# Malfoy/Brisk

Hardware: AMD Instinct MI355X
Metric: distinct k-mers indexed/sec (k=63,m=21) (higher is better)
Workload: dtype u64; 1 GPU; 1x MI355X: 50M synthetic 150 bp reads per GPU, k=63 m=21 b=14, uint8 counts, 15x coverage; reads_per_gpu=50000000, total_reads=50000000, part_bits=24, genome_len=500000000, parallelism=single GPU

## Files before the change

brisk_amd/csrc/brisk_insert.hip:

```cpp
#ifndef ARENA_CHUNK
#define ARENA_CHUNK 16384u
#endif
#ifndef INSERT_SLOTS
#define INSERT_SLOTS 8192u
#endif
#ifndef WI_WAVES_PER_EU
#define WI_WAVES_PER_EU 4
#endif
#ifdef BRISK_PHASE_PROF
__device__ unsigned long long g_phase[16];
#define PHASE_DECL unsigned long long ph_acc[12] = {0, 0, 0, 0, 0, 0, 0, 0, 0, 0, 0, 0}; unsigned long long ph_last = __builtin_amdgcn_s_memtime(); u32 dbg_cnt[16] = {0, 0, 0, 0, 0, 0, 0, 0, 0, 0, 0, 0, 0, 0, 0, 0};
#define PHASE(i) { const unsigned long long t_ = __builtin_amdgcn_s_memtime(); ph_acc[i] += t_ - ph_last; ph_last = t_; }
__device__ unsigned long long g_cnt[16];
#define PHASE_FLUSH { PHASE(10) if (threadIdx.x == 0) { _Pragma("unroll") for (int q_ = 0; q_ < 12; q_++) atomicAdd(&g_phase[q_], ph_acc[q_]); \
                                                         _Pragma("unroll") for (int q_ = 0; q_ < 16; q_++) atomicAdd(&g_cnt[q_], (unsigned long long)dbg_cnt[q_]); } }
#define CNT(i, v) dbg_cnt[i] += (v);
#else
#define PHASE_DECL
#define PHASE(i)
#define PHASE_FLUSH
#define CNT(i, v)
#endif
struct IndexDev {
    u64* keys;
// ... 152 lines not shown
    for (u32 it = 0; it < NI; it++) {
        const u32 i = it * 64 + lane;
        const u32 r = rix[it];
        const u64* c = s_rec + r * (NW ? NW + 1 : P.stride);
        const u64 hdr = c[NW ? NW : P.nw];
        const u32 j = i < ninst ? i - s_pref[r] : 0;
        const u128x key = make_key(P, hdr_bucket(hdr), record_kmer_lds<NW>(P, c, hdr_n(hdr), j), hdr_idx0(hdr) + j);
        klo[it] = key.lo;
        khi[it] = key.hi;
        hh[it] = hash_key32(key) & (tsize - 1);
        mult[it] = count8<SAT>(s_rmult[r]) << WI_CNT_SHIFT;
        if (i < ninst) {
            s_key[2 * i] = key.lo;
            s_key[2 * i + 1] = key.hi;
        }
    }
    wave_sync();
    u32 pending = 0;
#pragma unroll
    for (u32 it = 0; it < NI; it++)
        if (it * 64 + lane < ninst) pending |= 1u << it;
    while (__any(pending != 0)) {
        u32 old[NI];
#pragma unroll
        for (u32 it = 0; it < NI; it++) {
            old[it] = EMPTY_SLOT;
            if (pending >> it & 1) old[it] = atomicCAS(&s_tab[hh[it]], EMPTY_SLOT, (it * 64 + lane) | mult[it]);
        }
        u64 olo[NI], ohi[NI];
#pragma unroll
        for (u32 it = 0; it < NI; it++) {
            const u32 oi = old[it] == EMPTY_SLOT ? 0 : (old[it] & WI_IDX_MASK);
            olo[it] = s_key[2 * oi];
            ohi[it] = s_key[2 * oi + 1];
        }
#pragma unroll
        for (u32 it = 0; it < NI; it++) {
            if (pending >> it & 1) {
                if (old[it] == EMPTY_SLOT) {
                    pending &= ~(1u << it);
                } else if (olo[it] == klo[it] && ohi[it] == khi[it]) {
                    atomicAdd(&s_tab[hh[it]], mult[it]);
                    pending &= ~(1u << it);
                } else {
                    hh[it] = (hh[it] + 1) & (tsize - 1);
                }
            }
        }
    }
}

template <u32 NW>
struct RecGeom {
    static constexpr u32 CW = 2 * NW + 1;
    static constexpr u32 RS = 2 * NW + 3;
    static constexpr u32 INFO = 2 * NW + 1;
};
template <u32 NW>
__device__ __forceinline__ void store_rec_words(u32* dst, const RecRegs& rr, u32 info) {
    const u64 c0 = rr.w0, c1 = NW > 1 ? rr.w1 : 0, c2 = NW > 2 ? rr.w2 : 0, c3 = NW > 3 ? rr.w3 : 0;
    const u64 s0 = c0 << 6, s1 = (c1 << 6) | (c0 >> 58), s2 = (c2 << 6) | (c1 >> 58), s3 = (c3 << 6) | (c2 >> 58);
    const u32 top = (u32)((NW == 1 ? c0 : NW == 2 ? c1 : NW == 3 ? c2 : c3) >> 58);
    dst[0] = (u32)s0;
    dst[1] = (u32)(s0 >> 32);
    if (NW > 1) { dst[2] = (u32)s1; dst[3] = (u32)(s1 >> 32); }
    if (NW > 2) { dst[4] = (u32)s2; dst[5] = (u32)(s2 >> 32); }
    if (NW > 3) { dst[6] = (u32)s3; dst[7] = (u32)(s3 >> 32); }
    dst[2 * NW] = top;
    dst[RecGeom<NW>::INFO] = info;
    dst[RecGeom<NW>::INFO + 1] = 0;
}
template <u32 NIMAX>
struct LaneInst {
    u64 klo[NIMAX], khi[NIMAX];
    u32 hh[NIMAX];
    u32 won;
};
template <u32 NW, u32 KB, u32 SHIFT>
__device__ __forceinline__ void cut_key(const u32* base, u32 i, u32 ninst, u64* lo_out, u64* hi_out) {
    constexpr u32 INFO = RecGeom<NW>::INFO, KBITS = 2 * KB + 6;
    const u32 info = base[INFO];
    const u32 j = i < ninst ? i - (info & 0x3ffu) : 0;
    const u32 n = (info >> 10) & 0xffu;
    const u32 s = 2 * (n - 1 - j);
    const u32* wp = base + (s >> 5);
    const u32 sh = s & 31;
    const u32 w0 = wp[0], w1 = wp[1], w2 = wp[2], w3 = wp[3], w4 = wp[4];
    u32 k0 = __builtin_amdgcn_alignbit(w1, w0, sh), k1 = __builtin_amdgcn_alignbit(w2, w1, sh);
    u32 k2 = __builtin_amdgcn_alignbit(w3, w2, sh), k3 = __builtin_amdgcn_alignbit(w4, w3, sh);
    k0 = (k0 & ~0x3fu) | (((info >> 18) & 0xffu) + j);
    constexpr u32 m0 = KBITS >= 32 ? ~0u : (1u << KBITS) - 1, m1 = KBITS >= 64 ? ~0u : KBITS <= 32 ? 0u : (1u << (KBITS - 32)) - 1;
    constexpr u32 m2 = KBITS >= 96 ? ~0u : KBITS <= 64 ? 0u : (1u << (KBITS - 64)) - 1, m3 = KBITS >= 128 ? ~0u : KBITS <= 96 ? 0u : (1u << (KBITS - 96)) - 1;
    k0 &= m0; k1 &= m1; k2 &= m2; k3 &= m3;
    u64 lo = ((u64)k1 << 32) | k0, hi = ((u64)k3 << 32) | k2;
    if (SHIFT) {
        const u64 rl = (info >> 26) & ((1u << SHIFT) - 1);
        if (KBITS >= 64) hi |= rl << (KBITS - 64);
        else {
            lo |= rl << KBITS;
            if (KBITS + SHIFT > 64) hi |= rl >> (64 - KBITS);
        }
    }
    *lo_out = lo;
    *hi_out = hi;
}
template <u32 NI, u32 NW, u32 KB, u32 SHIFT, u32 NIMAX>
__device__ __forceinline__ void expand_words_distinct(u32 lane, u32 ninst, const u32* s_rw, const uint8_t* s_irec, LaneInst<NIMAX>& li) {
    static_assert(NI <= NIMAX, "instances per lane");
    u32 rix[NI];
    u32 won = 0;
#pragma unroll
    for (u32 it = 0; it < NI; it++) {
        const u32 i = it * 64 + lane;
        rix[it] = s_irec[i < ninst ? i : 0];
    }
#pragma unroll
    for (u32 it = 0; it < NI; it++) {
        const u32 i = it * 64 + lane;
        cut_key<NW, KB, SHIFT>(s_rw + rix[it] * RecGeom<NW>::RS, i, ninst, &li.klo[it], &li.khi[it]);
        if (i < ninst) won |= 1u << it;
    }
    li.won = won;
}
template <u32 NI, u32 NW, u32 KB, u32 SHIFT, u32 NIMAX, bool FOLD, bool SAT>
__device__ __forceinline__ void expand_and_dedupe_words(u32 lane, u32 ninst, u32 tsize, const u32* s_rw, const uint8_t* s_irec, const uint8_t* s_imult,
                                                        const u32* s_rmult, u64* s_key, u32* s_tab, u32* dbg_rounds, LaneInst<NIMAX>& li) {
    constexpr u32 RS = RecGeom<NW>::RS, KBITS = 2 * KB + 6;
    static_assert(KBITS + SHIFT <= 128 && SHIFT <= 6, "entry key: [routing id low bits | compacted k-mer | idx']");
    static_assert(NI <= NIMAX, "instances per lane");
    u64 (&klo)[NIMAX] = li.klo;
    u64 (&khi)[NIMAX] = li.khi;
    u32 (&hh)[NIMAX] = li.hh;
    u32 mult[NI];
    u32 rix[NI];
    u32 won = 0;
#pragma unroll
    for (u32 it = 0; it < NI; it++) {
        const u32 i = it * 64 + lane;
        rix[it] = s_irec[i < ninst ? i : 0];
    }
#pragma unroll
    for (u32 it = 0; it < NI; it++) {
        const u32 i = it * 64 + lane;
        u64 lo, hi;
        cut_key<NW, KB, SHIFT>(s_rw + rix[it] * RS, i, ninst, &lo, &hi);
        klo[it] = lo;
        khi[it] = hi;
        hh[it] = hash_key32(mk128(lo, hi)) & (tsize - 1);
        mult[it] = FOLD ? (u32)s_imult[i < ninst ? i : 0] << WI_CNT_SHIFT : count8<SAT>(s_rmult[rix[it]]) << WI_CNT_SHIFT;
        if (i < ninst) {
            s_key[2 * i] = lo;
            s_key[2 * i + 1] = hi;
        }
    }
    wave_sync();
    for (u32 w = 0; w * 64 < tsize; w++) s_tab[w * 64 + lane] = EMPTY_SLOT;
    wave_sync();
    u32 pending = 0;
#pragma unroll
    for (u32 it = 0; it < NI; it++)
        if (it * 64 + lane < ninst) pending |= 1u << it;
    while (__any(pending != 0)) {
        *dbg_rounds += NI;
        u32 old[NI];
#pragma unroll
        for (u32 it = 0; it < NI; it++) {
            old[it] = EMPTY_SLOT;
            if (pending >> it & 1) old[it] = atomicCAS(&s_tab[hh[it]], EMPTY_SLOT, (it * 64 + lane) | mult[it]);
        }
        u64 olo[NI], ohi[NI];
#pragma unroll
        for (u32 it = 0; it < NI; it++) {
            const u32 oi = old[it] == EMPTY_SLOT ? 0 : (old[it] & WI_IDX_MASK);
            olo[it] = s_key[2 * oi];
            ohi[it] = s_key[2 * oi + 1];
        }
#pragma unroll
        for (u32 it = 0; it < NI; it++) {
            if (pending >> it & 1) {
                if (old[it] == EMPTY_SLOT) {
                    pending &= ~(1u << it);
                    won |= 1u << it;
                } else if (olo[it] == klo[it] && ohi[it] == khi[it]) {
                    atomicAdd(&s_tab[hh[it]], mult[it]);
                    pending &= ~(1u << it);
                } else {
                    hh[it] = (hh[it] + 1) & (tsize - 1);
                }
            }
        }
    }
    li.won = won;
}

#define HDR_ID_MASK 0x0000ffffffffffffull
#define HDR_HAS_MULT (1ull << 56)
__device__ __forceinline__ bool dedupe_records(u32 stride, const RecRegs& rr, u32 my_mult, u32 nrec, u32 lane, const u64* s_rec, u32* s_rtab, u32* s_rmult) {
    s_rtab[lane] = EMPTY_SLOT;
    s_rtab[lane + 64] = EMPTY_SLOT;
    s_rmult[lane] = my_mult;
    wave_sync();
    bool dup = false;
    if (lane < nrec) {
        const u64 k1 = stride == 2 ? HDR_ID_MASK : ~0ull, k2 = stride == 3 ? HDR_ID_MASK : ~0ull, k3 = stride == 4 ? HDR_ID_MASK : ~0ull,
                  k4 = stride == 5 ? HDR_ID_MASK : ~0ull;
        const u64 w1 = rr.w1 & k1, w2 = rr.w2 & k2, w3 = rr.w3 & k3, w4 = rr.w4 & k4;
        const u64 z = rr.w0 ^ ((w1 << 17) | (w1 >> 47)) ^ ((w2 << 31) | (w2 >> 33)) ^ ((w3 << 47) | (w3 >> 17)) ^ w4;
        u32 h = ((((u32)z ^ (u32)(z >> 32)) * 0x9E3779B1u) >> 20) & (2 * WI_MAX_REC - 1);
        for (;;) {
            const u32 o = atomicCAS(&s_rtab[h], EMPTY_SLOT, lane);
            if (o == EMPTY_SLOT) break;
            const u64* oc = s_rec + o * stride;
            bool same = oc[0] == rr.w0 && (oc[1] & k1) == w1;
            if (stride > 2) same = same && (oc[2] & k2) == w2;
            if (stride > 3) same = same && (oc[3] & k3) == w3;
            if (stride > 4) same = same && (oc[4] & k4) == w4;
            if (same) {
                atomicAdd(&s_rmult[o], my_mult);
                dup = true;
                break;
            }
            h = (h + 1) & (2 * WI_MAX_REC - 1);
        }
    }
    return dup;
}

#ifndef WI_FOLD_TRIPS
#define WI_FOLD_TRIPS 16u
#endif
struct FoldFrame {
    W4 u, m;
    u32 rid;
    u32 rng;
    u32 s;
};
template <u32 NW, u32 KB>
__device__ __forceinline__ FoldFrame fold_frame(const RecRegs& rr, u64 hdr, u32 n, bool valid, u32 frame_end, u32 lane) {
    FoldFrame f;
    const u32 idx0 = hdr_idx0(hdr), end = idx0 + n, top = frame_end - idx0 + KB - 1;
    const bool ok = valid && n > 0 && end <= frame_end && top <= 32 * NW;
    const u32 lo_bits = ok ? 2 * (frame_end - end) : 0, hi_bits = ok ? 2 * top : 0;
    f.m = w4_andn(w4_mask(hi_bits), w4_mask(lo_bits));
    f.u = w4_and(w4_shl(W4{rr.w0, NW > 1 ? rr.w1 : 0, NW > 2 ? rr.w2 : 0, NW > 3 ? rr.w3 : 0}, lo_bits), f.m);
    f.rid = hdr_bucket(hdr);
    f.rng = idx0 | (end << 8);
    f.s = ok ? (n << 6) | (63 - lane) : 0;
    return f;
}
__device__ __forceinline__ u64 readlane64(u64 v, u32 a) {
    return ((u64)(u32)__builtin_amdgcn_readlane((int)(v >> 32), (int)a) << 32) | (u32)__builtin_amdgcn_readlane((int)v, (int)a);
}
template <u32 KB, u32 CW>
__device__ __forceinline__ u32 fold_core(const W4& u) {
    constexpr u32 LO = 2 * CW, N = 2 * (KB - CW), WI = LO / 64, BI = LO % 64;
    static_assert(CW < KB && N <= 28 && LO + N <= 256, "the core: the minimizer's nucleotides that are not cut out, m - b of them");
    const u64 w[5] = {u.w0, u.w1, u.w2, u.w3, 0};
    u64 v = w[WI] >> BI;
    if (BI + N > 64) v |= w[WI + 1] << (64 - BI);
    return (u32)v & ((1u << N) - 1);
}
template <u32 NW, bool DETECT = false>
__device__ __forceinline__ bool fold_records(const FoldFrame& f, u32 nrec, u32 lane, u32* lead, u32* off, u32* trips, u32 ck = 0, bool unsure = false, bool* clean = nullptr) {
    u32 sv = lane < nrec ? f.s : 0;
    bool folded = false;
    u32 dirty = unsure;
    *lead = lane;
    *off = 0;
    for (u32 t = 0; t < WI_FOLD_TRIPS; t++) {
        const u32 smax = (u32)__builtin_amdgcn_readlane((int)wave_incl_max_scan(sv), 63);
        if (smax == 0) break;
        *trips += 1;
        const u32 a = 63 - (smax & 63);
        const u32 rid_a = (u32)__builtin_amdgcn_readlane((int)f.rid, (int)a), rng_a = (u32)__builtin_amdgcn_readlane((int)f.rng, (int)a);
        const u32 i0 = f.rng & 0xffu, e = f.rng >> 8, i0a = rng_a & 0xffu, ea = rng_a >> 8;
#ifdef BRISK_NO_RECORD_FOLD
        bool in = sv != 0 && rid_a == f.rid && i0a == i0 && ea == e;
#else
        bool in = sv != 0 && rid_a == f.rid && i0a <= i0 && e <= ea;
#endif
        bool same = (readlane64(f.u.w0, a) & f.m.w0) == f.u.w0;
        if (NW > 1) same = same & ((readlane64(f.u.w1, a) & f.m.w1) == f.u.w1);
        if (NW > 2) same = same & ((readlane64(f.u.w2, a) & f.m.w2) == f.u.w2);
        if (NW > 3) same = same & ((readlane64(f.u.w3, a) & f.m.w3) == f.u.w3);
        in = in && same;
        if (in) {
            sv = 0;
            if (lane != a) {
                folded = true;
                *lead = a;
                *off = i0 - i0a;
            }
        }
        if (DETECT) {
            const u32 differs = ck ^ (u32)__builtin_amdgcn_readlane((int)ck, (int)a);
            const u32 meets = ((i0 - ea) & (i0a - e)) >> 31;
            dirty |= (differs == 0 && sv != 0) ? meets : 0u;
        }
    }
    if (DETECT) *clean = !__any((dirty | sv) != 0);
    return folded;
}

template <u32 MAXI, u32 NW, u32 KB, u32 SHIFT, bool SAT, bool LISTED = false>
__device__ __forceinline__ void insert_body(const BriskParams& PP, const RecSrc& src, const PartDesc* __restrict__ desc, u32 n_touched_all, const IndexDev& ix,
                                            u32* __restrict__ work_counter, const u32* __restrict__ list = nullptr, const u32* __restrict__ n_list = nullptr) {
    const u32 n_touched = LISTED ? min(*n_list, n_touched_all) : n_touched_all;
    u64* const rec = src.rec;
    BriskParams P = PP;
    if (NW) {
        P.nw = NW;
        P.stride = NW + 1;
        P.kb = KB;
        P.shift = SHIFT;
    }
    constexpr u32 TABLE = 2 * MAXI, TS = TABLE / 64, NI = MAXI / 64;
    constexpr u32 KW = NW ? (2 * KB + 6 + SHIFT <= 64 ? 1u : 2u) : 0u;
    constexpr bool FOLD = NW >= 3 && MAXI == WI_MAX_INST;
    static_assert(MAXI % 256 == 0 && MAXI <= 1024, "chunk size: whole 32-bit words of record marks per lane, 10-bit instance index");
    constexpr u32 REC_U64 = WI_MAX_REC * 5 > MAXI / 2 ? WI_MAX_REC * 5 : MAXI / 2;
    static_assert(NW == 0 || (WI_MAX_REC * RecGeom<NW ? NW : 1>::RS + 4) * 4 <= REC_U64 * 8, "shifted record words must fit the record buffer");
    constexpr bool TAB_OVER_REC = NW && TABLE * 4 <= REC_U64 * 8;
    constexpr u32 OFF_REC = 16 * MAXI, OFF_TAB = TAB_OVER_REC ? OFF_REC : OFF_REC + 8 * REC_U64, OFF_RTAB = TAB_OVER_REC ? OFF_REC + 8 * REC_U64 : OFF_TAB + 4 * TABLE;
    constexpr u32 OFF_RMULT = OFF_RTAB + 4 * 2 * WI_MAX_REC, OFF_IREC = OFF_RMULT + 4 * WI_MAX_REC, OFF_PREF = OFF_IREC + MAXI;
    constexpr u32 LDS_BYTES = NW ? OFF_PREF : OFF_PREF + 4 * (WI_MAX_REC + 1) + 4;
    __shared__ __attribute__((aligned(16))) unsigned char s_mem[LDS_BYTES];
    u64* s_key = (u64*)s_mem;
    u32* s_idiff = (u32*)s_mem;
    u64* s_rec = (u64*)(s_mem + OFF_REC);
    u32* s_rw = (u32*)s_rec;
    u32* s_tab = (u32*)(s_mem + OFF_TAB);
    u32* s_list = (u32*)s_rec;
    u32* s_rtab = (u32*)(s_mem + OFF_RTAB);
    u32* s_rmult = (u32*)(s_mem + OFF_RMULT);
    uint8_t* s_irec = s_mem + OFF_IREC;
    uint8_t* s_imult = s_mem + OFF_RTAB;
    static_assert(NW == 0 || MAXI <= 4 * 2 * WI_MAX_REC, "instance multiplicities fit the record table's bytes");
    u32* s_pref = (u32*)(s_mem + (NW ? 0 : OFF_PREF));

    const u32 lane = threadIdx.x;
    PHASE_DECL
    unsigned long long acur = ix.slot_cur[blockIdx.x], aend = ix.slot_end[blockIdx.x], garbage = 0;
    const u32 kbits = 2 * P.kb + 6;

    for (;;) {
        u32 t0 = 0;
        if (lane == 0) t0 = atomicAdd(work_counter, WI_BATCH);
        t0 = (u32)__builtin_amdgcn_readfirstlane((int)t0);
        if (t0 >= n_touched) break;
        const u32 t_end = min(t0 + WI_BATCH, n_touched);
        PartDesc d = desc[LISTED ? list[t0] : t0];
        RecRegs rr = load_part_recs(P, src, d.part, d.r_begin, d.r_begin, min(d.n_rec, (u32)WI_MAX_REC), lane);

        for (u32 t = t0; t < t_end; t++) {
            const u32 tn = t + 1;
            PartDesc dn{};
            if (tn < t_end) dn = desc[LISTED ? list[tn] : tn];
#define NEXT_PARTITION                                                                                                  \
    {                                                                                                                   \
        d = dn;                                                                                                         \
        if (tn < t_end) rr = load_part_recs(P, src, d.part, d.r_begin, d.r_begin, min(d.n_rec, (u32)WI_MAX_REC), lane); \
    }

            asm volatile("" ::"v"(rr.w0), "v"(rr.w1), "v"(rr.w2), "v"(rr.w3), "v"(rr.w4));
            do {
            if (ix.huge_at && d.n_inst > ix.huge_at) break;
            CNT(0, 1)
            const u32 part = d.part;
            u32 r_end = d.r_begin + d.n_rec;
            u32 n_exist = d.n_exist;
            u32 inst_left = d.n_inst;
            unsigned long long off = d.off;
            u32 cap = d.cap;
            u32 bm0 = 0, bm1 = 0;

            bool collapsed = false;
            if (MAXI > WI_MAX_INST && !src.bin_cap && d.n_rec > 2 * WI_MAX_REC) {
                u32 wr = d.r_begin;
                for (u32 rd = d.r_begin; rd < r_end; rd += WI_MAX_REC) {
                    const u32 avail = min(r_end - rd, (u32)WI_MAX_REC);
                    if (rd != d.r_begin) rr = load_rec_regs(P, rec, rd, avail, lane);
                    wave_sync();
                    if (lane < avail) {
                        u64* dst = s_rec + lane * P.stride;
                        dst[0] = rr.w0;
                        dst[1] = rr.w1;
                        if (P.stride > 2) dst[2] = rr.w2;
                        if (P.stride > 3) dst[3] = rr.w3;
                        if (P.stride > 4) dst[4] = rr.w4;
                    }
                    const u64 hdr_c = P.stride == 2 ? rr.w1 : P.stride == 3 ? rr.w2 : P.stride == 4 ? rr.w3 : rr.w4;
                    const u32 mult_c = (hdr_c & HDR_HAS_MULT) ? (u32)(hdr_c >> 48) & 0xffu : 1u;
                    const bool dup = dedupe_records(P.stride, rr, mult_c, avail, lane, s_rec, s_rtab, s_rmult);
                    wave_sync();
                    const bool keep = lane < avail && !dup;
                    const unsigned long long bal = __ballot(keep);
                    if (keep) {
                        u64* dst = rec + (u64)(wr + (u32)__popcll(bal & lanes_below(lane))) * P.stride;
                        const u64 keep_id = HDR_ID_MASK, mult = ((u64)count8<SAT>(s_rmult[lane]) << 48) | HDR_HAS_MULT;
                        dst[0] = rr.w0;
                        dst[1] = P.stride == 2 ? (rr.w1 & keep_id) | mult : rr.w1;
                        if (P.stride > 2) dst[2] = P.stride == 3 ? (rr.w2 & keep_id) | mult : rr.w2;
                        if (P.stride > 3) dst[3] = P.stride == 4 ? (rr.w3 & keep_id) | mult : rr.w3;
                        if (P.stride > 4) dst[4] = (rr.w4 & keep_id) | mult;
                    }
                    wr += (u32)__popcll(bal);
                }
                collapsed = true;
                r_end = wr;
                __builtin_amdgcn_fence(__ATOMIC_SEQ_CST, "workgroup");
                rr = load_rec_regs(P, rec, d.r_begin, min(r_end - d.r_begin, (u32)WI_MAX_REC), lane);
            }

            for (u32 rc = d.r_begin; rc < r_end;) {
                PHASE(0)
                CNT(1, 1)
                const u32 avail = min(r_end - rc, (u32)WI_MAX_REC);
                if (rc != d.r_begin) rr = load_part_recs(P, src, part, d.r_begin, rc, avail, lane);
                wave_sync();
                if (!FOLD && lane < avail) {
                    u64* dst = s_rec + lane * P.stride;
                    dst[0] = rr.w0;
                    dst[1] = rr.w1;
                    if (P.stride > 2) dst[2] = rr.w2;
                    if (P.stride > 3) dst[3] = rr.w3;
                    if (P.stride > 4) dst[4] = rr.w4;
                }
                const u64 my_hdr = P.stride == 2 ? rr.w1 : P.stride == 3 ? rr.w2 : P.stride == 4 ? rr.w3 : rr.w4;
                const u32 raw_n = lane < avail ? hdr_n(my_hdr) : 0;
                const u32 my_mult = (my_hdr & HDR_HAS_MULT) ? (u32)(my_hdr >> 48) & 0xffu : 1u;
                const u32 x0 = wave_incl_scan(raw_n, lane);
                const u32 rawfit = (u32)__popcll(__ballot(lane < avail && x0 <= MAXI));
                u32 nrec = avail, my_n = 0, x = 0, ninst = 0;
                u32 lead = lane, lead_off = 0, dbg_trips = 0;
                FoldFrame ff{};
                const u32 info_hi = (raw_n << 10) | (hdr_idx0(my_hdr) << 18) | ((hdr_bucket(my_hdr) & ((1u << SHIFT) - 1)) << 26);
                if (FOLD) {
                    ff = fold_frame<NW ? NW : 1, KB>(rr, my_hdr, raw_n, lane < avail, P.suff_reduc + P.w + 1, lane);
                    if (lane < avail) store_rec_words<NW ? NW : 1>(s_rw + lane * RecGeom<NW ? NW : 1>::RS, rr, 0);
                }
                for (int attempt = 0;; attempt++) {
                    CNT(2, 1)
                    bool dup;
                    if (FOLD) dup = fold_records<NW ? NW : 1>(ff, nrec, lane, &lead, &lead_off, &dbg_trips);
                    else dup = dedupe_records(P.stride, rr, my_mult, nrec, lane, s_rec, s_rtab, s_rmult);
                    my_n = (lane < nrec && !dup) ? raw_n : 0;
                    x = wave_incl_scan(my_n, lane);
                    ninst = __shfl(x, 63, 64);
                    if (ninst <= MAXI) break;
                    const u32 fit = (u32)__popcll(__ballot(lane < nrec && x <= MAXI));
                    nrec = (attempt >= 2 || fit <= rawfit) ? rawfit : min(fit, nrec - 1);
                    wave_sync();
                }
                PHASE(1)
                const u32 raw_inst = __shfl(x0, nrec - 1, 64);
                CNT(9, raw_inst)
                CNT(10, FOLD ? (u32)__popcll(__ballot(lane < nrec && my_n == 0 && raw_n != 0)) : 0u)
                CNT(11, dbg_trips)
                CNT(12, rc == d.r_begin && d.n_rec <= WI_MAX_REC && ninst > 64 && ninst <= 128 ? 1u : 0u)
                CNT(13, rc == d.r_begin && d.n_rec <= WI_MAX_REC && ninst > 128 && ninst <= 192 ? 1u : 0u)
                CNT(14, rc == d.r_begin && d.n_rec <= WI_MAX_REC && ninst > 192 ? 1u : 0u)
                CNT(15, rc == d.r_begin && d.n_rec > WI_MAX_REC ? 1u : 0u)
                const u32 m_first = FOLD ? (u32)__shfl(x - my_n, lead, 64) + lead_off : 0u;
                u32 tsize = 128;
                while (tsize < 4 * ninst && tsize < TABLE) tsize <<= 1;
                if (!NW) {
                    s_pref[lane + 1] = x;
                    if (lane == 0) s_pref[0] = 0;
#pragma unroll
                    for (u32 w = 0; w < TS; w++)
                        if (w * 64 < tsize) s_tab[w * 64 + lane] = EMPTY_SLOT;
                }
                {
                    u32* irec32 = (u32*)s_irec;
#pragma unroll
                    for (u32 q = 0; q < MAXI / 256; q++) irec32[q * 64 + lane] = 0;
                    if (FOLD) {
#pragma unroll
                        for (u32 q = 0; q < NI; q++) s_idiff[lane * NI + q] = 0;
                    }
                    wave_sync();
                    if (my_n) s_irec[x - my_n] = (uint8_t)(lane + 1);
                    if (FOLD && lane < nrec) {
                        atomicAdd(&s_idiff[m_first], my_mult);
                        if (m_first + raw_n < ninst) atomicAdd(&s_idiff[m_first + raw_n], 0u - my_mult);
                    }
                    wave_sync();
                    u32 wv[MAXI / 256], run = 0;
#pragma unroll
                    for (u32 q = 0; q < MAXI / 256; q++) {
                        wv[q] = irec32[lane * (MAXI / 256) + q];
                        run = op_max_u32(run, op_max_u32(op_max_u32(wv[q] & 0xff, (wv[q] >> 8) & 0xff), op_max_u32((wv[q] >> 16) & 0xff, wv[q] >> 24)));
                    }
                    if (FOLD) {
                        u32 mv[NI], tot = 0;
#pragma unroll
                        for (u32 q = 0; q < NI; q++) {
                            tot += s_idiff[lane * NI + q];
                            mv[q] = tot;
                        }
                        const u32 before = wave_incl_scan(tot, lane) - tot;
                        u32* mult32 = (u32*)s_imult;
#pragma unroll
                        for (u32 q = 0; q < NI / 4; q++)
                            mult32[lane * (NI / 4) + q] = count8<SAT>(mv[4 * q] + before) | (count8<SAT>(mv[4 * q + 1] + before) << 8) |
                                                          (count8<SAT>(mv[4 * q + 2] + before) << 16) |
                                                          ((SAT ? count8<SAT>(mv[4 * q + 3] + before) : mv[4 * q + 3] + before) << 24);
                    }
                    u32 carry = wave_prev_lane(wave_incl_max_scan(run));
#pragma unroll
                    for (u32 q = 0; q < MAXI / 256; q++) {
                        const u32 b0 = op_max_u32(carry, wv[q] & 0xff), b1 = op_max_u32(b0, (wv[q] >> 8) & 0xff);
                        const u32 b2 = op_max_u32(b1, (wv[q] >> 16) & 0xff), b3 = op_max_u32(b2, wv[q] >> 24);
                        carry = b3;
                        irec32[lane * (MAXI / 256) + q] = ((b0 - 1) & 0xff) | (((b1 - 1) & 0xff) << 8) | (((b2 - 1) & 0xff) << 16) | ((b3 - 1) << 24);
                    }
                }
                wave_sync();
                PHASE(2)
                u32 dbg_r = 0;
                LaneInst<NI> li;
                li.won = 0;
                CNT(3, (ninst + 63) / 64)
                CNT(4, ninst)
                CNT(5, nrec)
                if (NW) {
                    if (FOLD && lane < nrec) s_rw[lane * RecGeom<NW ? NW : 1>::RS + RecGeom<NW ? NW : 1>::INFO] = (x - my_n) | info_hi;
                    if (!FOLD && lane < nrec) store_rec_words<NW ? NW : 1>(s_rw + lane * RecGeom<NW ? NW : 1>::RS, rr, (x - my_n) | info_hi);
                    wave_sync();
                    if (ninst <= 64) expand_and_dedupe_words<1, NW ? NW : 1, KB, SHIFT, NI, FOLD, SAT>(lane, ninst, tsize, s_rw, s_irec, s_imult, s_rmult, s_key, s_tab, &dbg_r, li);
                    else if (ninst <= 128) expand_and_dedupe_words<2, NW ? NW : 1, KB, SHIFT, NI, FOLD, SAT>(lane, ninst, tsize, s_rw, s_irec, s_imult, s_rmult, s_key, s_tab, &dbg_r, li);
                    else if (ninst <= 192) expand_and_dedupe_words<3, NW ? NW : 1, KB, SHIFT, NI, FOLD, SAT>(lane, ninst, tsize, s_rw, s_irec, s_imult, s_rmult, s_key, s_tab, &dbg_r, li);
                    else if (NI <= 4 || ninst <= 256) expand_and_dedupe_words<4, NW ? NW : 1, KB, SHIFT, NI, FOLD, SAT>(lane, ninst, tsize, s_rw, s_irec, s_imult, s_rmult, s_key, s_tab, &dbg_r, li);
                    else expand_and_dedupe_words<NI, NW ? NW : 1, KB, SHIFT, NI, FOLD, SAT>(lane, ninst, tsize, s_rw, s_irec, s_imult, s_rmult, s_key, s_tab, &dbg_r, li);
                } else {
                    if (ninst <= 128) expand_and_dedupe<2, 0, SAT>(P, lane, ninst, tsize, s_rec, s_pref, s_irec, s_rmult, s_key, s_tab);
                    else if (NI <= 4 || ninst <= 256) expand_and_dedupe<4, 0, SAT>(P, lane, ninst, tsize, s_rec, s_pref, s_irec, s_rmult, s_key, s_tab);
                    else expand_and_dedupe<NI, 0, SAT>(P, lane, ninst, tsize, s_rec, s_pref, s_irec, s_rmult, s_key, s_tab);
                }
                wave_sync();
                CNT(8, dbg_r)
                PHASE(3)

                if (rc != d.r_begin) __builtin_amdgcn_fence(__ATOMIC_SEQ_CST, "workgroup");
                for (u32 e0 = 0; e0 < n_exist; e0 += 4 * 64) {
                    u64 klo[4], khi[4];
                    uint8_t cnt[4];
#pragma unroll
                    for (u32 q = 0; q < 4; q++) {
                        const u32 e = e0 + q * 64 + lane;
                        const unsigned long long at = off + (e < n_exist ? e : 0);
                        const u128x kq = load_key<KW>(ix, at);
                        klo[q] = kq.lo;
                        khi[q] = kq.hi;
                        cnt[q] = ix.counts[at];
                    }
#pragma unroll
                    for (u32 q = 0; q < 4; q++) {
                        const u32 e = e0 + q * 64 + lane;
                        if (e >= n_exist) continue;
                        u32 h = hash_key32(mk128(klo[q], khi[q])) & (tsize - 1);
                        for (;;) {
                            const u32 v = s_tab[h];
                            if (v == EMPTY_SLOT) break;
                            const u32 i = v & WI_IDX_MASK;
                            if (s_key[2 * i] == klo[q] && s_key[2 * i + 1] == khi[q]) {
                                ix.counts[off + e] = (uint8_t)count8<SAT>(cnt[q] + ((v & ~MATCHED_BIT) >> WI_CNT_SHIFT));
                                s_tab[h] = v | MATCHED_BIT;
                                break;
                            }
                            h = (h + 1) & (tsize - 1);
                        }
                    }
                }
                wave_sync();

                PHASE(5)
                u32 n_new = 0;
                u32 new_mask = 0, new_rank[NI], new_word[NI];
                if (NW) {
#pragma unroll
                    for (u32 it = 0; it < NI; it++) {
                        new_rank[it] = 0;
                        new_word[it] = 0;
                        if (it * 64 < ninst) {
                            const bool made = (li.won >> it) & 1;
                            if (made) new_word[it] = s_tab[li.hh[it]];
                            const bool is_new = made && !(new_word[it] & MATCHED_BIT);
                            const unsigned long long bal = __ballot(is_new);
                            new_rank[it] = n_new + (u32)__popcll(bal & lanes_below(lane));
                            if (is_new) new_mask |= 1u << it;
                            n_new += (u32)__popcll(bal);
                        }
                    }
                } else {
#pragma unroll
                    for (u32 w = 0; w < TS; w++) {
                        if (w * 64 < tsize) {
                            const u32 v = s_tab[w * 64 + lane];
                            const bool is_new = v != EMPTY_SLOT && !(v & MATCHED_BIT);
                            const unsigned long long bal = __ballot(is_new);
                            if (is_new) s_list[n_new + (u32)__popcll(bal & lanes_below(lane))] = v;
                            n_new += (u32)__popcll(bal);
                        }
                    }
                }
                wave_sync();
#ifndef INSERT_NO_EARLY_WAIT
                __builtin_amdgcn_s_waitcnt(0x0F70);
#endif

                PHASE(6)
                CNT(6, (n_new + 63) / 64)
                CNT(7, n_new)
                inst_left -= raw_inst;
                if (n_exist + n_new > cap) {
                    const unsigned long long want = grow_cap(n_exist + n_new + inst_left);
                    unsigned long long noff;
                    if (want > ARENA_CHUNK / 8) {
                        unsigned long long got = 0;
                        if (lane == 0) got = atomicAdd(ix.cursor, want);
                        noff = __shfl(got, 0, 64);
                    } else {
                        if (acur + want > aend) {
                            garbage += aend - acur;
                            unsigned long long got = 0;
                            if (lane == 0) got = atomicAdd(ix.cursor, (unsigned long long)ARENA_CHUNK);
                            acur = __shfl(got, 0, 64);
                            aend = acur + ARENA_CHUNK;
                        }
                        noff = acur;
                        acur += want;
                    }
                    if (noff + want > ix.arena_cap || ninst > MAXI) {
                        if (lane == 0) atomicOr(ix.err, ninst > MAXI ? 4u : 2u);
                        break;
                    }
                    garbage += cap;
                    cap = (u32)want;
                    for (u32 e = lane; e < n_exist; e += 64) {
                        move_key<KW>(ix, noff + e, off + e);
                        ix.counts[noff + e] = ix.counts[off + e];
                    }
                    off = noff;
                }
                PHASE(7)
                if (NW) {
#pragma unroll
                    for (u32 it = 0; it < NI; it++) {
                        if ((new_mask >> it) & 1) {
                            const unsigned long long at = off + n_exist + new_rank[it];
                            store_key<KW>(ix, at, li.klo[it], li.khi[it]);
                            ix.counts[at] = (uint8_t)count8<SAT>(new_word[it] >> WI_CNT_SHIFT);
                            const u32 bl = P.shift ? ((u32)shr128(mk128(li.klo[it], li.khi[it]), kbits).lo & ((1u << P.shift) - 1)) : 0;
                            const u32 bb = P.shift > 6 ? (bl >> (P.shift - 6)) : bl;
                            if (bb < 32) bm0 |= 1u << bb; else bm1 |= 1u << (bb - 32);
                        }
                    }
                } else {
                    for (u32 q = lane; q < n_new; q += 64) {
                        const u32 v = s_list[q];
                        const u32 i = v & WI_IDX_MASK;
                        const u64 klo2 = s_key[2 * i], khi2 = s_key[2 * i + 1];
                        const unsigned long long at = off + n_exist + q;
                        store_key<KW>(ix, at, klo2, khi2);
                        ix.counts[at] = (uint8_t)count8<SAT>(v >> WI_CNT_SHIFT);
                        const u32 bl = P.shift ? ((u32)shr128(mk128(klo2, khi2), kbits).lo & ((1u << P.shift) - 1)) : 0;
                        const u32 bb = P.shift > 6 ? (bl >> (P.shift - 6)) : bl;
                        if (bb < 32) bm0 |= 1u << bb; else bm1 |= 1u << (bb - 32);
                    }
                }
                n_exist += n_new;
                rc += nrec;
                PHASE(8)

            }
            if (P.shift <= 6) {
                bm0 = wave_or_all(bm0);
                if (P.shift == 6) bm1 = wave_or_all(bm1);
            }
            if (lane == 0) ix.dir[part] = DirEnt{off, n_exist, cap};
            if (P.shift <= 6 && lane < 2) {
                const u32 mask = lane == 0 ? bm0 : bm1;
                const u32 nb = 1u << P.shift;
                const u64 first = ((u64)part << P.shift) >> P.ext_bits;
                if (mask) {
                    if (nb >= 32) {
                        if (lane * 32 < nb && (!ix.bits_check || (ix.bucket_bits[(first >> 5) + lane] & mask) != mask)) atomicOr(&ix.bucket_bits[(first >> 5) + lane], mask);
                    } else if (lane == 0) {
                        const u32 bits = mask << (first & 31);
                        if (!ix.bits_check || (ix.bucket_bits[first >> 5] & bits) != bits) atomicOr(&ix.bucket_bits[first >> 5], bits);
                    }
                }
            }
            } while (0);
            NEXT_PARTITION
#undef NEXT_PARTITION
            PHASE(9)
        }
    }
    PHASE_FLUSH
    if (lane == 0) {
        ix.slot_cur[blockIdx.x] = acur;
        ix.slot_end[blockIdx.x] = aend;
        if (garbage) atomicAdd(&ix.stats[3], garbage);
    }
}


#ifndef WI_WAVES_PER_EU_FAST
#define WI_WAVES_PER_EU_FAST 5
#endif
template <u32 NW, u32 KB, u32 SHIFT, bool SAT = false>
__global__ void __launch_bounds__(64) __attribute__((amdgpu_waves_per_eu(WI_WAVES_PER_EU_FAST, 8))) k_insert_fast(BriskParams P, RecSrc src, const PartDesc* __restrict__ desc,
                                                                                                        u32 n_touched, IndexDev ix, u32* __restrict__ work_counter) {
    static_assert(NW > 0, "compile-time record geometry");
    insert_body<WI_MAX_INST, NW, KB, SHIFT, SAT>(P, src, desc, n_touched, ix, work_counter);
}
template <u32 NW, u32 KB, u32 SHIFT, bool SAT = false>
__global__ void __launch_bounds__(64) __attribute__((amdgpu_waves_per_eu(WI_WAVES_PER_EU_FAST, 8))) k_insert_fast_listed(BriskParams P, RecSrc src, const PartDesc* __restrict__ desc,
                                                                                                               u32 n_touched, IndexDev ix, u32* __restrict__ work_counter,
                                                                                                               const u32* __restrict__ list, const u32* __restrict__ n_list) {
    insert_body<WI_MAX_INST, NW, KB, SHIFT, SAT, true>(P, src, desc, n_touched, ix, work_counter, list, n_list);
}
template <u32 NW, u32 KB, u32 SHIFT, bool SAT = false>
__global__ void __launch_bounds__(64) __attribute__((amdgpu_waves_per_eu(WI_WAVES_PER_EU, 8))) k_insert(BriskParams P, RecSrc src, const PartDesc* __restrict__ desc,
                                               u32 n_touched, IndexDev ix, u32* __restrict__ work_counter) {
    insert_body<WI_MAX_INST, NW, KB, SHIFT, SAT>(P, src, desc, n_touched, ix, work_counter);
}
template <u32 NW, u32 KB, u32 SHIFT, bool SAT = false>
__global__ void __launch_bounds__(64) __attribute__((amdgpu_waves_per_eu(2, 8))) k_insert_big(BriskParams P, RecSrc src, const PartDesc* __restrict__ desc,
                                                                                         u32 n_touched, IndexDev ix, u32* __restrict__ work_counter) {
    insert_body<2 * WI_MAX_INST, NW, KB, SHIFT, SAT>(P, src, desc, n_touched, ix, work_counter);
}

#ifndef NI_LEAN
#define NI_LEAN 3
#endif
#ifndef WI_WAVES_PER_EU_FIRST
#define WI_WAVES_PER_EU_FIRST 6
#endif
#ifndef WI_WAVES_PER_EU_FIRST_MAX
#define WI_WAVES_PER_EU_FIRST_MAX 6
#endif
template <u32 NIL, u32 NW>
struct LeanLds {
    static constexpr u32 MAXI = 64 * NIL, TABLE = 512;
    static_assert((TABLE & (TABLE - 1)) == 0 && TABLE >= 2 * MAXI && TABLE <= 4 * MAXI, "probe table: a power of two, at most half full");
    static constexpr u32 REC_BYTES = (WI_MAX_REC * RecGeom<NW>::RS + 4) * 4;
    static constexpr u32 OFF_REC = 16 * MAXI;
    static constexpr u32 REGION = REC_BYTES > 4 * TABLE ? REC_BYTES : 4 * TABLE;
    static constexpr u32 OFF_IREC = OFF_REC + REGION, OFF_IMULT = OFF_IREC + MAXI, BYTES = OFF_IMULT + MAXI;
};
__device__ __forceinline__ unsigned long long first_lane64(unsigned long long v) {
    return ((unsigned long long)(u32)__builtin_amdgcn_readfirstlane((int)(v >> 32)) << 32) | (u32)__builtin_amdgcn_readfirstlane((int)v);
}
template <u32 NIL, u32 NW, u32 KB, u32 SHIFT, bool SAT>
__device__ __forceinline__ void insert_first_body(const BriskParams& P, const RecSrc& src, const PartDesc* __restrict__ desc, u32 n_touched, const IndexDev& ix,
                                                  u32* __restrict__ work_counter, u32* __restrict__ left_list, u32* __restrict__ n_left, u32* __restrict__ n_clean) {
    using L = LeanLds<NIL, NW>;
    constexpr u32 MAXI = L::MAXI, TABLE = L::TABLE, RS = RecGeom<NW>::RS, INFO = RecGeom<NW>::INFO, KBITS = 2 * KB + 6;
    constexpr u32 KW = KBITS + SHIFT <= 64 ? 1u : 2u;
    constexpr u32 CORE_K = 63, CORE_M = 21, CORE_B = 14, CW = CORE_K - CORE_M;
    static_assert(KB == CORE_K - CORE_B, "fold_core: the core of k63 m21 b14");
    static_assert(NIL == 2 || NIL == 3, "instance slots per lane");
    static_assert(NW >= 3 && SHIFT < 5, "the folding k63 geometries: at most 16 buckets per partition");
    static_assert(L::BYTES <= 13 * 512, "LDS per wave: 24 waves must fit a CU's 160 KiB");
    static_assert(4 * MAXI <= 16 * MAXI, "the multiplicity steps lie over the keys");
    static_assert(MAXI + (MAXI >> 2) + 8 <= ARENA_CHUNK / 8, "grow_cap(MAXI) is a small request: the host's arena reserve covers the tail a refill strands");
    __shared__ __attribute__((aligned(16))) unsigned char s_mem[L::BYTES];
    u64* s_key = (u64*)s_mem;
    u32* s_idiff = (u32*)s_mem;
    u32* s_rw = (u32*)(s_mem + L::OFF_REC);
    u32* s_tab = (u32*)(s_mem + L::OFF_REC);
    uint8_t* s_irec = s_mem + L::OFF_IREC;
    uint8_t* s_imult = s_mem + L::OFF_IMULT;

    const u32 lane = threadIdx.x;
    PHASE_DECL
    unsigned long long acur = first_lane64(ix.slot_cur[blockIdx.x]), aend = first_lane64(ix.slot_end[blockIdx.x]), garbage = 0;
    const u32 frame_end = P.suff_reduc + P.w + 1;
    const u32 core_from = (n_clean != nullptr && P.w == CW) ? P.suff_reduc : 0x100u;

    for (;;) {
        u32 t0 = 0;
        if (lane == 0) t0 = atomicAdd(work_counter, WI_BATCH);
        t0 = (u32)__builtin_amdgcn_readfirstlane((int)t0);
        if (t0 >= n_touched) break;
        const u32 t_end = min(t0 + WI_BATCH, n_touched);
        unsigned long long left_mask = 0;
        unsigned long long clean_mask = 0;
        PartDesc d = desc[t0];
        RecRegs rr = load_part_recs(P, src, d.part, d.r_begin, d.r_begin, min(d.n_rec, (u32)WI_MAX_REC), lane);

        for (u32 t = t0; t < t_end; t++) {
            const u32 tn = t + 1;
            PartDesc dn{};
            if (tn < t_end) dn = desc[tn];
            asm volatile("" ::"v"(rr.w0), "v"(rr.w1), "v"(rr.w2), "v"(rr.w3), "v"(rr.w4));
            do {
                if (ix.huge_at && d.n_inst > ix.huge_at) break;
                CNT(0, 1)
                if (d.n_exist | d.cap | (u32)(d.n_rec > WI_MAX_REC)) {
                    left_mask |= 1ull << (t - t0);
                    break;
                }
                PHASE(0)
                const u32 part = d.part, nrec = d.n_rec;
                const u64 my_hdr = NW == 3 ? rr.w3 : rr.w4;
                const u32 raw_n = lane < nrec ? hdr_n(my_hdr) : 0;
                const u32 my_mult = (my_hdr & HDR_HAS_MULT) ? (u32)(my_hdr >> 48) & 0xffu : 1u;
                const u32 info_hi = (raw_n << 10) | (hdr_idx0(my_hdr) << 18) | ((hdr_bucket(my_hdr) & ((1u << SHIFT) - 1)) << 26);
                const FoldFrame ff = fold_frame<NW, KB>(rr, my_hdr, raw_n, lane < nrec, frame_end, lane);
                wave_sync();
                if (lane < nrec) store_rec_words<NW>(s_rw + lane * RS, rr, 0);
                u32 lead = lane, lead_off = 0, dbg_trips = 0;
                const bool unsure = lane < nrec && (ff.s == 0 || hdr_idx0(my_hdr) < core_from);
                bool clean = false;
                const u32 ck = ((hdr_bucket(my_hdr) & ((1u << SHIFT) - 1)) << (2 * (KB - CW))) | fold_core<KB, CW>(ff.u);
                const bool dup = fold_records<NW, true>(ff, nrec, lane, &lead, &lead_off, &dbg_trips, ck, unsure, &clean);
#ifdef INSERT_ATTR_NOTABLE
                clean = true;
#endif
                const u32 my_n = (lane < nrec && !dup) ? raw_n : 0;
                const u32 x = wave_incl_scan(my_n, lane);
                const u32 ninst = (u32)__builtin_amdgcn_readlane((int)x, 63);
                if (ninst > MAXI) {
                    left_mask |= 1ull << (t - t0);
                    break;
                }
                PHASE(1)
                CNT(1, 1)
                const u32 m_first = (u32)__shfl(x - my_n, lead, 64) + lead_off;
                u32 tsize = 128;
                while (tsize < 4 * ninst && tsize < TABLE) tsize <<= 1;
                {
                    if (NIL == 2) ((uint16_t*)s_irec)[lane] = 0;
                    else {
#pragma unroll
                        for (u32 q = 0; q < NIL; q++) s_irec[q * 64 + lane] = 0;
                    }
#pragma unroll
                    for (u32 q = 0; q < NIL; q++) s_idiff[lane * NIL + q] = 0;
                    wave_sync();
                    if (my_n) s_irec[x - my_n] = (uint8_t)(lane + 1);
                    if (lane < nrec) {
                        atomicAdd(&s_idiff[m_first], my_mult);
                        if (m_first + raw_n < ninst) atomicAdd(&s_idiff[m_first + raw_n], 0u - my_mult);
                    }
                    wave_sync();
                    u32 mk[NIL], mv[NIL], run = 0, tot = 0;
                    if (NIL == 2) {
                        const u32 w = ((const uint16_t*)s_irec)[lane];
                        mk[0] = w & 0xff;
                        mk[1] = w >> 8;
                    } else {
#pragma unroll
                        for (u32 q = 0; q < NIL; q++) mk[q] = s_irec[lane * NIL + q];
                    }
#pragma unroll
                    for (u32 q = 0; q < NIL; q++) {
                        run = op_max_u32(run, mk[q]);
                        tot += s_idiff[lane * NIL + q];
                        mv[q] = tot;
                    }
                    const u32 before = wave_incl_scan(tot, lane) - tot;
                    u32 carry = wave_prev_lane(wave_incl_max_scan(run));
#pragma unroll
                    for (u32 q = 0; q < NIL; q++) {
                        carry = op_max_u32(carry, mk[q]);
                        mk[q] = (carry - 1) & 0xff;
                        mv[q] = count8<SAT>(mv[q] + before) & 0xff;
                    }
                    if (NIL == 2) {
                        ((uint16_t*)s_irec)[lane] = (uint16_t)(mk[0] | (mk[1] << 8));
                        ((uint16_t*)s_imult)[lane] = (uint16_t)(mv[0] | (mv[1] << 8));
                    } else {
#pragma unroll
                        for (u32 q = 0; q < NIL; q++) {
                            s_irec[lane * NIL + q] = (uint8_t)mk[q];
                            s_imult[lane * NIL + q] = (uint8_t)mv[q];
                        }
                    }
                    if (lane < nrec) s_rw[lane * RS + INFO] = (x - my_n) | info_hi;
                }
                wave_sync();
                PHASE(2)
                CNT(3, (ninst + 63) / 64)
                CNT(4, ninst)
                CNT(5, nrec)
                CNT(11, dbg_trips)
                u32 dbg_r = 0;
                LaneInst<NIL> li;
                li.won = 0;
                u32 n_new = 0, new_rank[NIL], new_word[NIL];
                if (clean) {
                    clean_mask |= 1ull << (t - t0);
                    u32 ln = lane;
                    asm volatile("" : "+v"(ln));
                    if (ninst <= 64) expand_words_distinct<1, NW, KB, SHIFT, NIL>(ln, ninst, s_rw, s_irec, li);
                    else if (NIL == 2 || ninst <= 128) expand_words_distinct<2, NW, KB, SHIFT, NIL>(ln, ninst, s_rw, s_irec, li);
                    else expand_words_distinct<NIL, NW, KB, SHIFT, NIL>(ln, ninst, s_rw, s_irec, li);
                    n_new = ninst;
#pragma unroll
                    for (u32 it = 0; it < NIL; it++) {
                        const u32 i = it * 64 + ln;
                        new_rank[it] = i;
                        new_word[it] = (u32)s_imult[i < ninst ? i : 0] << WI_CNT_SHIFT;
                    }
                    PHASE(3)
                } else {
                    if (ninst <= 64) expand_and_dedupe_words<1, NW, KB, SHIFT, NIL, true, SAT>(lane, ninst, tsize, s_rw, s_irec, s_imult, nullptr, s_key, s_tab, &dbg_r, li);
                    else if (NIL == 2 || ninst <= 128) expand_and_dedupe_words<2, NW, KB, SHIFT, NIL, true, SAT>(lane, ninst, tsize, s_rw, s_irec, s_imult, nullptr, s_key, s_tab, &dbg_r, li);
                    else expand_and_dedupe_words<NIL, NW, KB, SHIFT, NIL, true, SAT>(lane, ninst, tsize, s_rw, s_irec, s_imult, nullptr, s_key, s_tab, &dbg_r, li);
                    wave_sync();
                    CNT(8, dbg_r)
                    PHASE(3)
#pragma unroll
                    for (u32 it = 0; it < NIL; it++) {
                        new_rank[it] = 0;
                        new_word[it] = 0;
                        if (it * 64 < ninst) {
                            const bool made = (li.won >> it) & 1;
                            if (made) new_word[it] = s_tab[li.hh[it]];
                            const unsigned long long bal = __ballot(made);
                            new_rank[it] = n_new + (u32)__popcll(bal & lanes_below(lane));
                            n_new += (u32)__popcll(bal);
                        }
                    }
                }
                wave_sync();
#ifndef INSERT_NO_EARLY_WAIT
                __builtin_amdgcn_s_waitcnt(0x0F70);
#endif
                PHASE(6)
                CNT(7, n_new)
                unsigned long long off = d.off;
                u32 cap = 0;
                if (n_new) {
                    const unsigned long long want = grow_cap(n_new);
                    if (acur + want > aend) {
                        garbage += aend - acur;
                        unsigned long long got = 0;
                        if (lane == 0) got = atomicAdd(ix.cursor, (unsigned long long)ARENA_CHUNK);
                        acur = first_lane64(got);
                        aend = acur + ARENA_CHUNK;
                    }
                    if (acur + want > ix.arena_cap) {
                        if (lane == 0) atomicOr(ix.err, 2u);
                        n_new = 0;
                    } else {
                        off = acur;
                        acur += want;
                        cap = (u32)want;
                    }
                }
                PHASE(7)
                u32 bm0 = 0;
#pragma unroll
                for (u32 it = 0; it < NIL; it++) {
                    if (it * 64 < ninst && ((li.won >> it) & 1) && n_new) {
                        const unsigned long long at = off + new_rank[it];
                        store_key<KW>(ix, at, li.klo[it], li.khi[it]);
                        ix.counts[at] = (uint8_t)count8<SAT>(new_word[it] >> WI_CNT_SHIFT);
                        const u32 bl = SHIFT ? ((u32)shr128(mk128(li.klo[it], li.khi[it]), KBITS).lo & ((1u << SHIFT) - 1)) : 0;
                        bm0 |= 1u << bl;
                    }
                }
                PHASE(8)
                bm0 = wave_or_all(bm0);
                if (lane == 0) {
                    ix.dir[part] = DirEnt{off, n_new, cap};
                    const u64 first = ((u64)part << SHIFT) >> P.ext_bits;
                    const u32 bits = bm0 << (first & 31);
                    if (bits && (!ix.bits_check || (ix.bucket_bits[first >> 5] & bits) != bits)) atomicOr(&ix.bucket_bits[first >> 5], bits);
                }
            } while (0);
            d = dn;
            if (tn < t_end) rr = load_part_recs(P, src, d.part, d.r_begin, d.r_begin, min(d.n_rec, (u32)WI_MAX_REC), lane);
            PHASE(9)
        }
        if (left_mask) {
            const u32 n = (u32)__popcll(left_mask);
            u32 at = 0;
            if (lane == 0) at = atomicAdd(n_left, n);
            at = (u32)__builtin_amdgcn_readfirstlane((int)at);
            u32 ln = lane;
            asm volatile("" : "+v"(ln));
            if ((left_mask >> ln) & 1) left_list[at + (u32)__popcll(left_mask & lanes_below(ln))] = t0 + ln;
        }
        if (clean_mask && n_clean && lane == 0) atomicAdd(n_clean, (u32)__popcll(clean_mask));
    }
    PHASE_FLUSH
    if (lane == 0) {
        ix.slot_cur[blockIdx.x] = acur;
        ix.slot_end[blockIdx.x] = aend;
        if (garbage) atomicAdd(&ix.stats[3], garbage);
    }
}
template <u32 NW, u32 KB, u32 SHIFT, bool SAT = false, u32 NIL = NI_LEAN>
__global__ void __launch_bounds__(64) __attribute__((amdgpu_waves_per_eu(WI_WAVES_PER_EU_FIRST, WI_WAVES_PER_EU_FIRST_MAX))) k_insert_first(BriskParams P, RecSrc src, const PartDesc* __restrict__ desc,
                                                                                                          u32 n_touched, IndexDev ix, u32* __restrict__ work_counter,
                                                                                                          u32* __restrict__ left_list, u32* __restrict__ n_left, u32* __restrict__ n_clean) {
    insert_first_body<NIL, NW, KB, SHIFT, SAT>(P, src, desc, n_touched, ix, work_counter, left_list, n_left, n_clean);
}

__global__ void __launch_bounds__(256) k_bucket_bits(BriskParams P, IndexDev ix, u32 n_parts) {
    const u32 kbits = 2 * P.kb + 6;
    for (u32 part = blockIdx.x; part < n_parts; part += gridDim.x) {
        const u32 cnt = ix.dir[part].cnt;
        const unsigned long long off = ix.dir[part].off;
        for (u32 e = threadIdx.x; e < cnt; e += blockDim.x) {
            const u128x key = load_key(ix, off + e);
            const u32 bucket = (part << P.shift) | ((u32)shr128(key, kbits).lo & ((1u << P.shift) - 1));
            const u32 bit = 1u << (bucket & 31);
            if (!(ix.bucket_bits[bucket >> 5] & bit)) atomicOr(&ix.bucket_bits[bucket >> 5], bit);
        }
    }
}

__global__ void __launch_bounds__(256) k_stats(const DirEnt* __restrict__ dir, u64 n_parts, const u32* __restrict__ bits, u64 n_words,
                                               unsigned long long* out ) {
    __shared__ unsigned long long s_a[4], s_b[4], s_c[4];
    unsigned long long a = 0, b = 0, c = 0;
    const u64 stride = (u64)gridDim.x * blockDim.x;
    for (u64 i = (u64)blockIdx.x * blockDim.x + threadIdx.x; i < n_parts; i += stride) {
        const u32 v = dir[i].cnt;
        a += v;
        c = v > c ? v : c;
    }
    for (u64 i = (u64)blockIdx.x * blockDim.x + threadIdx.x; i < n_words; i += stride) b += __popc(bits[i]);
    for (int o = 32; o > 0; o >>= 1) {
        a += __shfl_down(a, o, 64);
        b += __shfl_down(b, o, 64);
        const unsigned long long c2 = __shfl_down(c, o, 64);
        c = c2 > c ? c2 : c;
    }
    if ((threadIdx.x & 63) == 0) {
        s_a[threadIdx.x >> 6] = a;
        s_b[threadIdx.x >> 6] = b;
        s_c[threadIdx.x >> 6] = c;
    }
    __syncthreads();
    if (threadIdx.x == 0) {
        atomicAdd(&out[0], s_a[0] + s_a[1] + s_a[2] + s_a[3]);
        atomicAdd(&out[1], s_b[0] + s_b[1] + s_b[2] + s_b[3]);
        unsigned long long m = s_c[0];
        for (int i = 1; i < 4; i++) m = s_c[i] > m ? s_c[i] : m;
        atomicMax(&out[2], m);
    }
}


#define HG_THREADS 1024u
#define HG_INST 2048u
#define HG_TAB 4096u
#define HG_LIVE 0x80000000u
#define HG_EXIST 0x40000000u
#define HG_MULT 0x3fffffffu
__device__ __forceinline__ const u64* huge_rec(const BriskParams& P, const RecSrc& src, const PartDesc& d, u32 i) {
    if (!src.bin_cap) return src.rec + (u64)(d.r_begin + i) * P.stride;
    return i < src.bin_cap ? src.rec + ((u64)d.part * src.bin_cap + i) * P.stride : src.ovf + ((u64)d.r_begin + i - src.bin_cap) * P.stride;
}
__device__ __forceinline__ u32 block_incl_scan(u32 v, u32* s_wsum, u32* total) {
    const u32 lane = threadIdx.x & 63, wid = threadIdx.x >> 6;
    u32 x = v;
    for (int o = 1; o < 64; o <<= 1) {
        const u32 y = __shfl_up(x, o, 64);
        if ((int)lane >= o) x += y;
    }
    __syncthreads();
    if (lane == 63) s_wsum[wid] = x;
    __syncthreads();
    u32 before = 0, all = 0;
    for (u32 i = 0; i < HG_THREADS / 64; i++) {
        const u32 c = s_wsum[i];
        if (i < wid) before += c;
        all += c;
    }
    *total = all;
    return x + before;
}
template <bool SAT>
__global__ void __launch_bounds__(HG_THREADS) k_insert_huge(BriskParams P, RecSrc src, const PartDesc* __restrict__ desc, const u32* __restrict__ huge_list,
                                                            const u32* __restrict__ n_huge, IndexDev ix) {
    __shared__ u64 s_key[2 * HG_INST];
    __shared__ u32 s_tab[HG_TAB];
    __shared__ u32 s_cnt[HG_INST];
    __shared__ u32 s_pref[HG_THREADS + 1];
    __shared__ u32 s_wsum[HG_THREADS / 64];
    __shared__ u32 s_nkeys, s_bm[2], s_fail;
    __shared__ unsigned long long s_noff;
    const u32 tid = threadIdx.x;
    const u32 kbits = 2 * P.kb + 6;
    for (u32 hi = blockIdx.x; hi < *n_huge; hi += gridDim.x) {
        const PartDesc d = desc[huge_list[hi]];
        u32 n_exist = d.n_exist, cap = d.cap, inst_left = d.n_inst;
        unsigned long long off = d.off, garbage = 0;
        if (tid < 2) s_bm[tid] = 0;
        if (tid == 0) s_fail = 0;
        bool failed = false;
        for (u32 rc = 0; rc < d.n_rec && !failed;) {
            const u32 avail = min(d.n_rec - rc, HG_THREADS);
            u32 my_n = 0;
            if (tid < avail) my_n = hdr_n(huge_rec(P, src, d, rc + tid)[P.nw]);
            u32 all;
            const u32 x = block_incl_scan(my_n, s_wsum, &all);
            s_pref[tid + 1] = x;
            if (tid == 0) {
                s_pref[0] = 0;
                s_nkeys = 0;
            }
            for (u32 i = tid; i < HG_TAB; i += HG_THREADS) s_tab[i] = EMPTY_SLOT;
            u32 nrec;
            (void)block_incl_scan(tid < avail && x <= HG_INST ? 1u : 0u, s_wsum, &nrec);
            __syncthreads();
            const u32 ninst = s_pref[nrec];
            for (u32 i = tid; i < ninst; i += HG_THREADS) {
                u32 lo = 0, hi2 = nrec;
                while (hi2 - lo > 1) {
                    const u32 mid = (lo + hi2) >> 1;
                    if (s_pref[mid] <= i) lo = mid; else hi2 = mid;
                }
// ... 125 lines not shown
```

Before: 31.17 billion k-mers/s.

## Add hashed grouped record folding with shared-memory leader election

Adds a grouped fold path that hashes each record's core key into a shared-memory slot and elects a leader per slot with atomicMax. Each round can then fold many distinct groups in parallel, instead of the existing per-leader iterative fold. Lanes fetch the leader's frame through ds_bpermute. If rounds run out, a lane is unsure, or leftovers remain, the code falls back to the original fold_records. It is meant to cut the number of serial fold trips per wave, at the cost of LDS atomics, extra syncs, and possibly doing the work twice when it falls back.

```diff
diff --git a/brisk_amd/csrc/brisk_insert.hip b/brisk_amd/csrc/brisk_insert.hip
--- a/brisk_amd/csrc/brisk_insert.hip
+++ b/brisk_amd/csrc/brisk_insert.hip
@@ -478,6 +478,66 @@
     return folded;
 }
 
+#ifndef FOLD_GROUPED
+#define FOLD_GROUPED 1
+#endif
+#ifdef INSERT_ATTR_ONEROUND
+#define FOLD_GROUPED_TRIPS 1u
+#else
+#define FOLD_GROUPED_TRIPS WI_FOLD_TRIPS
+#endif
+__device__ __forceinline__ u32 fold_slot(u32 ck) { return (ck * 0x9E3779B1u) >> 26; }
+__device__ __forceinline__ u32 lane_fetch(u32 v, u32 a4) { return (u32)__builtin_amdgcn_ds_bpermute((int)a4, (int)v); }
+__device__ __forceinline__ u64 lane_fetch64(u64 v, u32 a4) { return ((u64)lane_fetch((u32)(v >> 32), a4) << 32) | lane_fetch((u32)v, a4); }
+template <u32 NW>
+__device__ __forceinline__ bool fold_records_grouped(const FoldFrame& f, u32 nrec, u32 lane, u32* s_slot, u32* lead, u32* off, bool* folded_out, u32* trips, u32 ck, bool unsure,
+                                                     bool* clean) {
+    static_assert(WI_FOLD_TRIPS < (1u << 18), "[round | n | 63 - lane] in 32 bits: n < 256, so sv < 1 << 14");
+    if (__any(unsure)) return false;
+    u32 sv = lane < nrec ? f.s : 0;
+    bool folded = false;
+    u32 dirty = 0, heads = 0;
+    *lead = lane;
+    *off = 0;
+    u32* my_slot = s_slot + fold_slot(ck);
+    s_slot[lane] = 0;
+    wave_sync();
+    for (u32 t = 1; t <= FOLD_GROUPED_TRIPS; t++) {
+        if (!__any(sv != 0) || heads > WI_FOLD_TRIPS) break;
+        *trips += 1;
+        const u32 mine = (t << 14) | sv;
+        if (sv != 0) atomicMax(my_slot, mine);
+        wave_sync();
+        const u32 top = *my_slot;
+        heads += (u32)__popcll(__ballot(sv != 0 && top == mine));
+        const u32 a = 63 - (top & 63), a4 = a << 2;
+        const u32 rng_a = lane_fetch(f.rng, a4), ck_a = lane_fetch(ck, a4);
+        const u32 i0 = f.rng & 0xffu, e = f.rng >> 8, i0a = rng_a & 0xffu, ea = rng_a >> 8;
+        bool in = sv != 0 && ck_a == ck && i0a <= i0 && e <= ea;
+        bool same = (lane_fetch64(f.u.w0, a4) & f.m.w0) == f.u.w0;
+        if (NW > 1) same = same & ((lane_fetch64(f.u.w1, a4) & f.m.w1) == f.u.w1);
+        if (NW > 2) same = same & ((lane_fetch64(f.u.w2, a4) & f.m.w2) == f.u.w2);
+        if (NW > 3) same = same & ((lane_fetch64(f.u.w3, a4) & f.m.w3) == f.u.w3);
+        in = in && same;
+        if (in) {
+            sv = 0;
+            if (lane != a) {
+                folded = true;
+                *lead = a;
+                *off = i0 - i0a;
+            }
+        }
+        const u32 meets = ((i0 - ea) & (i0a - e)) >> 31;
+        dirty |= (ck_a == ck && sv != 0) ? meets : 0u;
+    }
+#ifndef INSERT_ATTR_ONEROUND
+    if (heads > WI_FOLD_TRIPS || __any(sv != 0)) return false;
+#endif
+    *clean = !__any(dirty != 0);
+    *folded_out = folded;
+    return true;
+}
+
 template <u32 MAXI, u32 NW, u32 KB, u32 SHIFT, bool SAT, bool LISTED = false>
 __device__ __forceinline__ void insert_body(const BriskParams& PP, const RecSrc& src, const PartDesc* __restrict__ desc, u32 n_touched_all, const IndexDev& ix,
                                             u32* __restrict__ work_counter, const u32* __restrict__ list = nullptr, const u32* __restrict__ n_list = nullptr) {
@@ -994,7 +1054,9 @@
                 const bool unsure = lane < nrec && (ff.s == 0 || hdr_idx0(my_hdr) < core_from);
                 bool clean = false;
                 const u32 ck = ((hdr_bucket(my_hdr) & ((1u << SHIFT) - 1)) << (2 * (KB - CW))) | fold_core<KB, CW>(ff.u);
-                const bool dup = fold_records<NW, true>(ff, nrec, lane, &lead, &lead_off, &dbg_trips, ck, unsure, &clean);
+                bool dup = false;
+                if (!FOLD_GROUPED || !fold_records_grouped<NW>(ff, nrec, lane, (u32*)s_mem, &lead, &lead_off, &dup, &dbg_trips, ck, unsure, &clean))
+                    dup = fold_records<NW, true>(ff, nrec, lane, &lead, &lead_off, &dbg_trips, ck, unsure, &clean);
 #ifdef INSERT_ATTR_NOTABLE
                 clean = true;
 #endif
```

After: 33.82 billion k-mers/s, median of 6. +8.5%, better.
